# aerius-labs/zksnap-circuits-halo2

Hardware: AMD Instinct MI355X
Metric: BN254 G1 MSM Mpoints/sec (higher is better)
Workload: dtype u32x9 (254-bit modular integer, radix 2^29); 1 GPU; BN254 G1 MSM, 2^20 random points/scalars per GPU (BASELINE configs[1]), point-range sharded x1, inputs resident in HBM, bases registered once (prepared fixed-base table, as under ParamsKZG::commit); points_per_gpu=1048576, parallelism=point-range shard x1 + all_gather(96 B) + fold

## Files before the change

zksnap_circuits_halo2_amd/csrc/msm.hip:

```cpp
#include <hip/hip_runtime.h>
#include <atomic>
#include <cstdint>
#include <cstdio>
#include <cstring>
#include <cstdlib>
#include <mutex>
#include "ec_quad.hpp"
#include "fe_inverse.hpp"
#include "zkhip_internal.hpp"

namespace zkhip {

static inline size_t align_up(size_t v, size_t a) { return (v + a - 1) / a * a; }

constexpr int FINE_BITS = 12;
constexpr int MAX_GROUPS = 128;
constexpr int MAX_WIDE_W = 16;
struct win_layout { int c, W, narrow; };
__host__ __device__ __forceinline__ int win_bits(const win_layout& L, int w) { return w < L.W - L.narrow ? L.c : L.c - 1; }
__host__ __device__ __forceinline__ int win_off(const win_layout& L, int w) { const int full = L.W - L.narrow; return w <= full ? w * L.c : full * L.c + (w - full) * (L.c - 1); }
static int msm_narrow_windows(int c, int W) {
  if (c <= 16) return 0;
  const int narrow = W * c - 256;
  return narrow > 0 && narrow <= W ? narrow : 0;
}
constexpr int MAX_TASK_LEN = 128;
constexpr int TASK_SHIFT = 6;

__device__ __forceinline__ xyzz load_xyzz(const uint32_t* base, size_t idx) {
  const uint4* q = reinterpret_cast<const uint4*>(base + idx * 36);
  uint32_t w[36];
#pragma unroll
  for (int i = 0; i < 9; i++) {
    uint4 v = q[i];
    w[4 * i] = v.x; w[4 * i + 1] = v.y; w[4 * i + 2] = v.z; w[4 * i + 3] = v.w;
  }
  xyzz r;
#pragma unroll
  for (int i = 0; i < 9; i++) { r.X.l[i] = w[i]; r.Y.l[i] = w[9 + i]; r.ZZ.l[i] = w[18 + i]; r.ZZZ.l[i] = w[27 + i]; }
  return r;
}

__device__ __forceinline__ void store_xyzz(uint32_t* base, size_t idx, const xyzz& a) {
  uint32_t w[36];
#pragma unroll
  for (int i = 0; i < 9; i++) { w[i] = a.X.l[i]; w[9 + i] = a.Y.l[i]; w[18 + i] = a.ZZ.l[i]; w[27 + i] = a.ZZZ.l[i]; }
  uint4* q = reinterpret_cast<uint4*>(base + idx * 36);
#pragma unroll
  for (int i = 0; i < 9; i++) q[i] = make_uint4(w[4 * i], w[4 * i + 1], w[4 * i + 2], w[4 * i + 3]);
}

__device__ __forceinline__ xyzz xyzz_shfl_xor(const xyzz& a, int mask) {
  xyzz r;
#pragma unroll
  for (int i = 0; i < NL; i++) {
    r.X.l[i] = (uint32_t)__shfl_xor((int)a.X.l[i], mask, 64);
    r.Y.l[i] = (uint32_t)__shfl_xor((int)a.Y.l[i], mask, 64);
    r.ZZ.l[i] = (uint32_t)__shfl_xor((int)a.ZZ.l[i], mask, 64);
    r.ZZZ.l[i] = (uint32_t)__shfl_xor((int)a.ZZZ.l[i], mask, 64);
  }
  return r;
}

__device__ __forceinline__ fe load_fe9_generic(const uint32_t* p, size_t idx) {
  fe r;
#pragma unroll
  for (int i = 0; i < 9; i++) r.l[i] = p[idx * 9 + i];
  return r;
}
__device__ __forceinline__ void store_fe9_generic(uint32_t* p, size_t idx, const fe& a) {
#pragma unroll
  for (int i = 0; i < 9; i++) p[idx * 9 + i] = a.l[i];
}

__global__ void __launch_bounds__(256) k_digits(const uint32_t* __restrict__ scalars, int16_t* __restrict__ digits,
                                                uint32_t n, uint32_t n_pad, int c, int W, uint32_t K, size_t scalar_stride, int narrow) {
  const size_t idx = (size_t)blockIdx.x * blockDim.x + threadIdx.x;
  if (idx >= (size_t)K * n_pad) return;
  const uint32_t kb = (uint32_t)(idx / n_pad), i = (uint32_t)(idx % n_pad);
  digits += (size_t)kb * n_pad;
  const size_t row = (size_t)K * n_pad;
  if (i >= n) {
    for (int win = 0; win < W; win++) digits[(size_t)win * row + i] = 0;
    return;
  }
  uint32_t w[8];
  load_words(scalars + ((size_t)kb * scalar_stride + i) * 8, w);
  fe c32;
#pragma unroll
  for (int k = 0; k < NL; k++) c32.l[k] = FrParams::FROM_EXT_CANON[k];
  fe s = fe_canon_lt2p<FrParams>(fe_mul<FrParams>(c32, fe_unpack<0>(w)));
  fe_pack(s, w);
  const win_layout lay{c, W, narrow};
  uint32_t carry = 0;
  for (int win = 0; win < W; win++) {
    const int bit = win_off(lay, win), cw = win_bits(lay, win);
    const uint32_t half = 1u << (cw - 1), mask = (1u << cw) - 1;
    uint32_t v = 0;
    if (bit < 256) {
      int wi = bit >> 5, sh = bit & 31;
      uint64_t two = w[wi];
      if (wi + 1 < 8) two |= (uint64_t)w[wi + 1] << 32;
      v = (uint32_t)(two >> sh) & mask;
    }
    v += carry;
    int32_t d;
    if (v >= half) { d = (int32_t)v - (int32_t)(1u << cw); carry = 1; } else { d = (int32_t)v; carry = 0; }
    digits[(size_t)win * row + i] = (int16_t)d;
  }
}

__global__ void __launch_bounds__(1024) k_digits_wide(const uint32_t* __restrict__ scalars, int32_t* __restrict__ digits, uint32_t n, uint32_t n_pad,
                                                       int c, int W, uint32_t* __restrict__ gcount, int narrow) {
  __shared__ uint32_t cnt[MAX_WIDE_W * MAX_GROUPS];
  for (uint32_t t = threadIdx.x; t < (uint32_t)W * MAX_GROUPS; t += blockDim.x) cnt[t] = 0;
  __syncthreads();
  const win_layout lay{c, W, narrow};
  for (uint32_t i = blockIdx.x * blockDim.x + threadIdx.x; i < n_pad; i += gridDim.x * blockDim.x) {
    if (i >= n) {
      for (int win = 0; win < W; win++) digits[(size_t)win * n_pad + i] = 0;
      continue;
    }
    uint32_t w[8];
    load_words(scalars + (size_t)i * 8, w);
    fe c32;
#pragma unroll
    for (int k = 0; k < NL; k++) c32.l[k] = FrParams::FROM_EXT_CANON[k];
    fe sv = fe_canon_lt2p<FrParams>(fe_mul<FrParams>(c32, fe_unpack<0>(w)));
    fe_pack(sv, w);
    uint32_t carry = 0;
    for (int win = 0; win < W; win++) {
      const int bit = win_off(lay, win), cw = win_bits(lay, win);
      const uint32_t half = 1u << (cw - 1), mask = (1u << cw) - 1;
      uint32_t v = 0;
      if (bit < 256) {
        const int wi = bit >> 5, sh = bit & 31;
        uint64_t two = w[wi];
        if (wi + 1 < 8) two |= (uint64_t)w[wi + 1] << 32;
        v = (uint32_t)(two >> sh) & mask;
      }
      v += carry;
      int32_t d;
      if (v >= half) { d = (int32_t)v - (int32_t)(1u << cw); carry = 1; } else { d = (int32_t)v; carry = 0; }
      digits[(size_t)win * n_pad + i] = d;
      if (d != 0) atomicAdd(&cnt[win * MAX_GROUPS + (((uint32_t)(d < 0 ? -d : d) - 1) >> FINE_BITS)], 1u);
    }
  }
  __syncthreads();
  for (uint32_t t = threadIdx.x; t < (uint32_t)W * MAX_GROUPS; t += blockDim.x)
    if (cnt[t]) atomicAdd(&gcount[t], cnt[t]);
}

namespace glv {
__device__ constexpr uint32_t G1[3] = {0xc7e0b3d7u, 0xd91d232eu, 0x2u};
__device__ constexpr uint32_t G2[5] = {0x391eb18eu, 0x7a7bd9d4u, 0xa773d2cfu, 0x4ccef014u, 0x2u};
__device__ constexpr uint32_t A1[2] = {0x94d213e3u, 0x89d32568u};
__device__ constexpr uint32_t A2[4] = {0x1221250bu, 0x0be4e154u, 0xeeb859fdu, 0x6f4d8248u};
__device__ constexpr uint32_t NB1[4] = {0x7d4f1128u, 0x8211bbebu, 0xeeb859fcu, 0x6f4d8248u};
__device__ constexpr uint32_t BETA_EXT[8] = {0xd782e155u, 0x71930c11u, 0xffbe3323u, 0xa6bb947cu, 0xd4741444u, 0xaa303344u, 0x26594943u, 0x2c3b3f0du};

template <int NA, int NB, int NO>
// ... 820 lines not shown

__device__ __forceinline__ xyzz workgroup_sum_128(xyzz acc, uint32_t* __restrict__ xch) {
#pragma unroll 1
  for (uint32_t half = 64; half >= 1; half >>= 1) {
    __syncthreads();
    if (threadIdx.x >= half && threadIdx.x < 2 * half) store_xyzz(xch, threadIdx.x - half, acc);
    __syncthreads();
    if (threadIdx.x < half) acc = xyzz_add(acc, load_xyzz(xch, threadIdx.x));
  }
  return acc;
}

__device__ __forceinline__ void combine_heavy_buckets(uint32_t wg, const uint32_t* __restrict__ task_off, uint32_t* __restrict__ partials,
                                                      uint32_t* __restrict__ buckets, const uint32_t* __restrict__ heavy_count,
                                                      const uint2* __restrict__ heavy, uint32_t heavy_cap, uint32_t* __restrict__ heavy_done,
                                                      uint32_t* __restrict__ xch , uint32_t quad_max) {
  __shared__ uint32_t is_last;
  const uint32_t nh = min(*heavy_count, heavy_cap);
  for (uint32_t i = wg; i < nh; i += HEAVY_WGS) {
    const uint2 e = heavy[i];
    const uint32_t k = e.x, sl = e.y, t = task_off[k], m = task_off[k + 1] - t;
    const uint32_t P = (m + HEAVY_SLICE - 1) / HEAVY_SLICE, lo = sl * HEAVY_SLICE, hi = min(m, lo + HEAVY_SLICE);
    if (m <= quad_max) {
      const uint32_t q = threadIdx.x & 3, quad = threadIdx.x >> 2;
      xyzz acc = xyzz_identity();
#pragma unroll 1
      for (uint32_t j = quad; j < m; j += 32) acc = xyzz_add_quad(acc, load_xyzz(partials, t + j), q);
#pragma unroll 1
      for (int mask = 4; mask < 64; mask <<= 1) acc = xyzz_add_quad(acc, xyzz_shfl_xor(acc, mask), q);
      __syncthreads();
      if (threadIdx.x == 64) store_xyzz(xch, 0, acc);
      __syncthreads();
      if (threadIdx.x < 4) {
        acc = xyzz_add_quad(acc, load_xyzz(xch, 0), q);
        if (q == 0) store_xyzz(buckets, k, acc);
      }
      continue;
    }
    xyzz acc = xyzz_identity();
#pragma unroll 1
    for (uint32_t j = lo + threadIdx.x; j < hi; j += 128) acc = xyzz_add(acc, load_xyzz(partials, t + j));
    acc = workgroup_sum_128(acc, xch);
    if (P == 1) {
      if (threadIdx.x == 0) store_xyzz(buckets, k, acc);
      continue;
    }
    if (threadIdx.x == 0) {
      store_xyzz(partials, t + lo, acc);
      __threadfence();
      is_last = atomicAdd(&heavy_done[i - sl], 1u) == P - 1;
    }
    __syncthreads();
    if (!is_last) continue;
    __threadfence();
    acc = xyzz_identity();
#pragma unroll 1
    for (uint32_t j = threadIdx.x; j < P; j += 128) acc = xyzz_add(acc, load_xyzz(partials, t + j * HEAVY_SLICE));
    acc = workgroup_sum_128(acc, xch);
    if (threadIdx.x == 0) store_xyzz(buckets, k, acc);
  }
}

template <int COMBINE_LANES>
__global__ void __launch_bounds__(128) k_combine_seq(const uint32_t* __restrict__ task_off, uint32_t nbuckets,
                                                     uint32_t* __restrict__ partials, uint32_t* __restrict__ buckets,
                                                     uint32_t seq_parts, uint32_t blocks, const uint32_t* __restrict__ heavy_count,
                                                     const uint2* __restrict__ heavy, uint32_t heavy_cap, uint32_t* __restrict__ heavy_done, uint32_t quad_max) {
  __shared__ __attribute__((aligned(16))) uint32_t xch[64 * 36];
  if (blockIdx.x >= blocks) { combine_heavy_buckets(blockIdx.x - blocks, task_off, partials, buckets, heavy_count, heavy, heavy_cap, heavy_done, xch, quad_max); return; }
  const uint32_t gid = blockIdx.x * blockDim.x + threadIdx.x;
  const uint32_t k = gid / COMBINE_LANES, q = gid % COMBINE_LANES;
  const bool live = k < nbuckets;
  xyzz acc = xyzz_identity();
  uint32_t m = 0;
  if (live) {
    const uint32_t t = task_off[k];
    m = task_off[k + 1] - t;
    const uint32_t left = (m == 1 || m > seq_parts) ? 0u : m;
#pragma unroll 1
    for (uint32_t j = q; j < left; j += COMBINE_LANES) acc = xyzz_add(acc, load_xyzz(partials, t + j));
  }
#pragma unroll 1
  for (int mask = 1; mask < COMBINE_LANES; mask <<= 1) acc = xyzz_add(acc, xyzz_shfl_xor(acc, mask));
  if (live && q == 0 && m != 1 && m <= seq_parts) store_xyzz(buckets, k, acc);
}

template <int COMBINE_LANES>
__global__ void __launch_bounds__(128) k_combine_seq_quad(const uint32_t* __restrict__ task_off, uint32_t nbuckets,
                                                          uint32_t* __restrict__ partials, uint32_t* __restrict__ buckets,
                                                          uint32_t seq_parts, uint32_t blocks, const uint32_t* __restrict__ heavy_count,
                                                          const uint2* __restrict__ heavy, uint32_t heavy_cap, uint32_t* __restrict__ heavy_done, uint32_t quad_max) {
  __shared__ __attribute__((aligned(16))) uint32_t xch[64 * 36];
  if (blockIdx.x >= blocks) { combine_heavy_buckets(blockIdx.x - blocks, task_off, partials, buckets, heavy_count, heavy, heavy_cap, heavy_done, xch, quad_max); return; }
  const uint32_t gid = blockIdx.x * blockDim.x + threadIdx.x;
  const uint32_t q = gid & 3, lane = (gid >> 2) % COMBINE_LANES, k = (gid >> 2) / COMBINE_LANES;
  const bool live = k < nbuckets;
  xyzz acc = xyzz_identity();
  uint32_t m = 0;
  if (live) {
    const uint32_t t = task_off[k];
    m = task_off[k + 1] - t;
    const uint32_t left = (m == 1 || m > seq_parts) ? 0u : m;
#pragma unroll 1
    for (uint32_t j = lane; j < left; j += COMBINE_LANES) acc = xyzz_add_quad(acc, load_xyzz(partials, t + j), q);
  }
#pragma unroll 1
  for (int mask = 1; mask < COMBINE_LANES; mask <<= 1) acc = xyzz_add_quad(acc, xyzz_shfl_xor(acc, 4 * mask), q);
  if (live && lane == 0 && q == 0 && m != 1 && m <= seq_parts) store_xyzz(buckets, k, acc);
}

__global__ void __launch_bounds__(128) k_pyramid_step(const uint32_t* __restrict__ in, uint32_t* __restrict__ out,
                                                      uint32_t N, int s, uint32_t in_stride, uint32_t out_stride) {
  const uint32_t per_win = N / 2 + (uint32_t)s * (N / 4);
  const int win = blockIdx.y;
  const uint32_t* wi = in + (size_t)win * in_stride * 36;
  uint32_t* wo = out + (size_t)win * out_stride * 36;
#pragma unroll 1
  for (uint32_t tid = blockIdx.x * blockDim.x + threadIdx.x; tid < per_win; tid += gridDim.x * blockDim.x) {
    uint32_t ia, ib;
    if (tid < N / 2) {
      ia = 2 * tid; ib = 2 * tid + 1;
    } else {
      uint32_t r = tid - N / 2;
      uint32_t l = r / (N / 4), u = r % (N / 4);
      if ((int)l == s - 1) { ia = 4 * u + 1; ib = 4 * u + 3; }
      else { ia = N + l * (N / 2) + 2 * u; ib = ia + 1; }
    }
    store_xyzz(wo, tid, xyzz_add(load_xyzz(wi, ia), load_xyzz(wi, ib)));
  }
}

__global__ void __launch_bounds__(128) k_pyramid_step_quad(const uint32_t* __restrict__ in, uint32_t* __restrict__ out,
                                                           uint32_t N, int s, uint32_t in_stride, uint32_t out_stride) {
  const uint32_t per_win = N / 2 + (uint32_t)s * (N / 4);
  const uint32_t gid = blockIdx.x * blockDim.x + threadIdx.x;
  const uint32_t tid = gid >> 2, q = gid & 3;
  if (tid >= per_win) return;
  const int win = blockIdx.y;
  const uint32_t* wi = in + (size_t)win * in_stride * 36;
  uint32_t* wo = out + (size_t)win * out_stride * 36;
  uint32_t ia, ib;
  if (tid < N / 2) {
    ia = 2 * tid; ib = 2 * tid + 1;
  } else {
    uint32_t r = tid - N / 2;
    uint32_t l = r / (N / 4), u = r % (N / 4);
    if ((int)l == s - 1) { ia = 4 * u + 1; ib = 4 * u + 3; }
    else { ia = N + l * (N / 2) + 2 * u; ib = ia + 1; }
  }
  const xyzz r = xyzz_add_quad(load_xyzz(wi, ia), load_xyzz(wi, ib), q);
  if (q == 0) store_xyzz(wo, tid, r);
}

__global__ void __launch_bounds__(64) k_window_horner(const uint32_t* __restrict__ in, uint32_t in_stride, int nz,
                                                      uint32_t* __restrict__ winsum, int W) {
  const int gid = blockIdx.x * blockDim.x + threadIdx.x;
  const int win = gid >> 5, lane = gid & 31;
  xyzz acc = xyzz_identity();
  if (win < W) {
    const uint32_t* wi = in + (size_t)win * in_stride * 36;
    int dbl = 0;
    if (lane < nz) { acc = load_xyzz(wi, 2 + lane); dbl = lane; }
    else if (lane == nz) { acc = load_xyzz(wi, 1); dbl = nz; }
    else if (lane == nz + 1) acc = xyzz_add(load_xyzz(wi, 0), load_xyzz(wi, 1));
#pragma unroll 1
    for (int i = 0; i < dbl; i++) acc = xyzz_dbl(acc);
  }
#pragma unroll 1
  for (int mask = 1; mask < 32; mask <<= 1) acc = xyzz_add(acc, xyzz_shfl_xor(acc, mask));
  if (win < W && lane == 0) store_xyzz(winsum, win, acc);
}

__global__ void __launch_bounds__(128) k_window_horner_quad(const uint32_t* __restrict__ in, uint32_t in_stride, int nz,
                                                            uint32_t* __restrict__ winsum, uint32_t* __restrict__ jac_out) {
  __shared__ __attribute__((aligned(16))) uint32_t xch[36];
  const int win = blockIdx.x, term = threadIdx.x >> 2;
  const uint32_t q = threadIdx.x & 3;
  const uint32_t* wi = in + (size_t)win * in_stride * 36;
  xyzz acc = xyzz_identity();
  int dbl = 0;
  if (term < nz) { acc = load_xyzz(wi, 2 + term); dbl = term; }
  else if (term == nz) { acc = load_xyzz(wi, 1); dbl = nz; }
  else if (term == nz + 1) acc = xyzz_add_quad(load_xyzz(wi, 0), load_xyzz(wi, 1), q);
#pragma unroll 1
  for (int i = 0; i < dbl; i++) acc = xyzz_dbl_quad(acc, q);
#pragma unroll 1
  for (int mask = 4; mask < 64; mask <<= 1) acc = xyzz_add_quad(acc, xyzz_shfl_xor(acc, mask), q);
  if (threadIdx.x == 64) store_xyzz(xch, 0, acc);
  __syncthreads();
  if (threadIdx.x < 4) {
    acc = xyzz_add_quad(acc, load_xyzz(xch, 0), q);
    if (q == 0) {
      if (jac_out) store_jacobian(acc, jac_out + (size_t)win * 24);
      else store_xyzz(winsum, win, acc);
    }
  }
}

__global__ void __launch_bounds__(64) k_fold(const uint32_t* __restrict__ winsum, int W, int c, uint32_t* __restrict__ out) {
  if (threadIdx.x >= 4 || blockIdx.x != 0) return;
  const uint32_t q = threadIdx.x;
  xyzz acc = load_xyzz(winsum, W - 1);
  for (int w = W - 2; w >= 0; w--) {
#pragma unroll 1
    for (int i = 0; i < c; i++) acc = xyzz_dbl_quad(acc, q);
    acc = xyzz_add_quad(acc, load_xyzz(winsum, w), q);
  }
  if (q == 0) store_jacobian(acc, out);
}

__global__ void __launch_bounds__(64) k_store_results(const uint32_t* __restrict__ winsum, uint32_t K, uint32_t* __restrict__ out) {
  const uint32_t k = blockIdx.x * blockDim.x + threadIdx.x;
  if (k < K) store_jacobian(load_xyzz(winsum, k), out + (size_t)k * 24);
}

__global__ void __launch_bounds__(64) k_sum_jacobian(const uint32_t* __restrict__ in, int m, uint32_t* __restrict__ out, uint32_t stride) {
  const uint32_t q = threadIdx.x & 3;
  const int grp = threadIdx.x >> 2;
  in += (size_t)blockIdx.x * 24;
  out += (size_t)blockIdx.x * 24;
  xyzz acc = xyzz_identity();
  for (int i = grp; i < m; i += 16) acc = xyzz_add_quad(acc, load_jacobian(in + (size_t)i * stride * 24), q);
#pragma unroll 1
  for (int mask = 4; mask < 64; mask <<= 1) {
    if ((mask >> 2) >= m && mask > 4) break;
    acc = xyzz_add_quad(acc, xyzz_shfl_xor(acc, mask), q);
  }
  if (threadIdx.x == 0) store_jacobian(acc, out);
}

static bool msm_top_window_is_degenerate(int c) {
  const int W = (256 + c - 1) / c, top_bits = 254 - (W - 1) * c;
  return top_bits > 0 && top_bits < 6;
}

static inline int msm_windows(int c, bool glv) {
  if (!glv) return (256 + c - 1) / c;
  return (128 + c - 1) / c + ((c == 2 || c == 4) ? 1 : 0);
}

int msm_pick_window(size_t n) {
  int best = 16;
  double best_cost = 1e300;
  for (int c = 2; c <= 16; c++) {
    const int Wi = msm_windows(c, true), top_bits = 127 - (Wi - 1) * c;
    if (top_bits > 0 && top_bits < 6) continue;
    const double cost = (double)Wi * (10.0 * (double)(2 * n) + 28.0 * (double)(1u << (c - 1)));
    if (cost < best_cost) { best_cost = cost; best = c; }
  }
  return best;
}


constexpr int MAX_WINDOW_PREPARED = 20;

int msm_pick_window_prepared(size_t n) {
  const bool large = n >= ((size_t)1 << 20);
  int best = 2;
  double best_cost = 1e300;
  for (int c = 2; c <= MAX_WINDOW_PREPARED; c++) {
    const double W = (256 + c - 1) / c, buckets = (double)(1u << (c - 1));
    if (msm_top_window_is_degenerate(c) && c <= 16) continue;
    if (c > 16 && !large) continue;
    if (c == 17) continue;
    double cost;
    if (!large) cost = W * 10.0 * (double)n + 28.0 * buckets;
    else {
      const double eff = c == 20 ? 1.0 : (c == 19 ? 1.13 : (c == 18 ? 1.06 : 1.07));
      cost = W * (10.0 * eff + 1.0) * (double)n + 39.0 * buckets + 1.1e6 * (double)(c - 2) + 13.0e6;
    }
    if (cost < best_cost) { best_cost = cost; best = c; }
  }
  if (n >= ((size_t)1 << 14) && n < ((size_t)3 << 14)) best = 15;
  return best;
}

struct msm_layout {
  uint32_t task_shift;
  size_t max_tasks;
  void* digits;
  uint32_t* stage_ref; uint16_t* stage_fine;
  char* zero_lo; size_t zero_bytes;
  uint32_t *gcounters, *counters, *count, *sorted, *offset, *cursor, *task_off, *bsum1, *bsum2;
  task_t* tasks; uint4* order;
  uint32_t *partials, *pyrA, *pyrB, *winsum;
  uint32_t* endo;
  int combine_lanes;
  uint32_t seq_parts;
  uint2* heavy; uint32_t heavy_cap;
  uint32_t* heavy_done;
  size_t total;
};

static uint32_t msm_task_shift(size_t entries , size_t NB, size_t xyzz_bytes = 144) {
  uint32_t task_shift = TASK_SHIFT;
  if ((entries >> 7) >= ((size_t)3 << 16)) task_shift = 7;
  const bool g2 = xyzz_bytes == 288;
  if ((entries >> TASK_SHIFT) < ((size_t)1 << (g2 ? 14 : 17))) {
    const double occ = (double)entries / (double)NB;
    double best = 1e300;
    for (uint32_t sh = 2; sh <= (uint32_t)TASK_SHIFT; sh++) {
      const double L = (double)(1u << sh), parts = occ / L;
      const double est = 5.0 * L + (g2 ? 15.0 : 10.0) * (parts > 1.0 ? parts - 1.0 : 0.0);
      if (est < best) { best = est; task_shift = sh; }
    }
  }
  return task_shift;
}

constexpr size_t GLV_TWO_LEVEL_MIN = (size_t)1 << 18;
constexpr size_t PREP_TWO_LEVEL_MIN = (size_t)1 << 16;
static bool msm_two_level(int c, bool glv, size_t n_in, bool shared_buckets, size_t K) {
  if (c > 16) return true;
  if (c != 16 || K != 1) return false;
  if (glv) return n_in >= GLV_TWO_LEVEL_MIN;
  return shared_buckets && n_in >= PREP_TWO_LEVEL_MIN;
}

static msm_layout msm_lay_out(char* base, size_t n_in, size_t K, int c, bool prepared, size_t xyzz_bytes = 144, bool glv = false) {
  msm_layout L;
  const size_t n = glv ? 2 * n_in : n_in;
  const size_t W = (size_t)msm_windows(c, glv), B = (size_t)1 << (c - 1), WB = prepared ? K : W, NB = WB * B;
  const bool wide = msm_two_level(c, glv, n_in, prepared, K);
  const size_t nk = n * K, entries = W * nk;
  const size_t n_pad = (n + 7) & ~(size_t)7;
  L.task_shift = msm_task_shift(entries, NB, xyzz_bytes);
  L.max_tasks = (entries >> L.task_shift) + NB + 1;
  const double parts_avg = (double)entries / (double)NB / (double)(1u << L.task_shift);
  L.combine_lanes = parts_avg <= 2.0 ? 1 : (parts_avg <= 4.0 ? 2 : (parts_avg <= 12.0 ? 4 : 8));
  L.seq_parts = 16u * (uint32_t)L.combine_lanes;
  L.heavy_cap = (uint32_t)(std::min<size_t>(L.max_tasks / (L.seq_parts + 1) + 1, NB) + L.max_tasks / HEAVY_SLICE + 1);
  char* p = base;
  auto carve = [&](size_t bytes) { void* r = p; p += align_up(bytes, 256); return r; };
  L.digits = carve(W * K * n_pad * (wide ? sizeof(int32_t) : sizeof(int16_t)));
  L.stage_ref = wide ? (uint32_t*)carve(entries * sizeof(uint32_t)) : nullptr;
  L.stage_fine = wide ? (uint16_t*)carve(entries * sizeof(uint16_t)) : nullptr;
  L.zero_lo = p;
  L.gcounters = wide ? (uint32_t*)carve(32768) : nullptr;
  L.counters = (uint32_t*)carve(2048);
  L.count = (uint32_t*)carve((NB + 1) * sizeof(uint32_t));
  L.heavy_done = (uint32_t*)carve((size_t)L.heavy_cap * sizeof(uint32_t));
  L.zero_bytes = (size_t)(p - L.zero_lo);
  L.sorted = (uint32_t*)carve(entries * sizeof(uint32_t));
  L.offset = (uint32_t*)carve((NB + 1) * sizeof(uint32_t));
  L.cursor = (uint32_t*)carve((NB + 1) * sizeof(uint32_t));
  L.task_off = (uint32_t*)carve((NB + 1) * sizeof(uint32_t));
  L.heavy = (uint2*)carve((size_t)L.heavy_cap * sizeof(uint2));
  L.bsum1 = (uint32_t*)carve((NB / SCAN_TILE + 2) * sizeof(uint32_t));
// ... 29 lines not shown
                    size_t xyzz_bytes, void* ws, size_t ws_bytes, hipStream_t stream, msm_tasks_view* out, bool glv) {
  const uint32_t K = (uint32_t)batch;
  const bool wide = msm_two_level(c, glv, n_in, shared_buckets, batch);
  const int W = msm_windows(c, glv);
  if (glv && (K != 1 || c > 16 || shared_buckets)) { set_error("msm: GLV digits are for one vector of the general path"); return ZKHIP_EINVAL; }
  const size_t n = glv ? 2 * n_in : n_in;
  const uint32_t B = 1u << (c - 1);
  const int WB = shared_buckets ? (int)K : W;
  const uint32_t NB = (uint32_t)WB * B;
  if ((size_t)W * n * K >= (1ull << 32) || (size_t)WB * B >= (1ull << 31)) { set_error("msm: W*n*batch overflows 32-bit slot index"); return ZKHIP_EINVAL; }
  if (c > 16 && (!shared_buckets || K != 1)) { set_error("msm: windows above 16 bits need one shared bucket set"); return ZKHIP_EINVAL; }
  if (wide && !shared_buckets && (size_t)W * (B >> FINE_BITS) > (size_t)MAX_GROUPS) { set_error("msm: two-level sort: %d windows x %u groups exceed %d", W, B >> FINE_BITS, MAX_GROUPS); return ZKHIP_EINVAL; }
  if (wide && W > MAX_WIDE_W) { set_error("msm: %d windows of %d bits exceed the wide path's %d", W, c, MAX_WIDE_W); return ZKHIP_EINVAL; }
  const msm_layout lay = msm_lay_out((char*)ws, n_in, K, c, shared_buckets, xyzz_bytes, glv);
  if (ws_bytes < lay.total) { set_error("msm: workspace too small (%zu < %zu bytes)", ws_bytes, lay.total); return ZKHIP_EINVAL; }
  const uint32_t task_shift = lay.task_shift;
  const uint32_t n_pad = (uint32_t)((n + 7) & ~(size_t)7);
  void* const digits = lay.digits;
  uint32_t* const stage_ref = lay.stage_ref;
  uint16_t* const stage_fine = lay.stage_fine;
  uint32_t *const gcounters = lay.gcounters, *const counters = lay.counters, *const count = lay.count, *const sorted = lay.sorted,
           *const offset = lay.offset, *const cursor = lay.cursor, *const task_off = lay.task_off, *const bsum1 = lay.bsum1, *const bsum2 = lay.bsum2;
  task_t* const tasks = lay.tasks;
  uint4* const order = lay.order;

  prof_begin(stream);
  HIPCHK(hipMemsetAsync(lay.zero_lo, 0, lay.zero_bytes, stream));
  const size_t sstride = K > 1 ? scalar_stride : n;
  const size_t nk = n * K, max_tasks = lay.max_tasks;
  (void)nk; (void)max_tasks;
  const unsigned dblocks = (unsigned)(((size_t)K * n_pad + 255) / 256);
  const int narrow = (shared_buckets && !glv) ? msm_narrow_windows(c, W) : 0;
  if (glv && wide) hipLaunchKernelGGL(k_digits_glv<int32_t>, dim3((unsigned)((std::max<size_t>(n_in, 8) + 255) / 256)), dim3(256), 0, stream, d_scalars, (int32_t*)digits, (uint32_t)n_in, n_pad, c, W);
  else if (glv) hipLaunchKernelGGL(k_digits_glv<int16_t>, dim3((unsigned)((std::max<size_t>(n_in, 8) + 255) / 256)), dim3(256), 0, stream, d_scalars, (int16_t*)digits, (uint32_t)n_in, n_pad, c, W);
  else if (wide) {
    const unsigned wg_cap = n_pad > (1u << 21) ? 1024u : 512u;
    const unsigned wblocks = (unsigned)std::min<size_t>(((size_t)n_pad + 1023) / 1024, wg_cap);
    hipLaunchKernelGGL(k_digits_wide, dim3(wblocks), dim3(1024), 0, stream, d_scalars, (int32_t*)digits, (uint32_t)n, n_pad, c, W, gcounters + 1024, narrow);
  }
  else hipLaunchKernelGGL(k_digits, dim3(dblocks), dim3(256), 0, stream, d_scalars, (int16_t*)digits, (uint32_t)n, n_pad, c, W, K, sstride, 0);
  prof_mark(stream, "digits");
  uint32_t chunks = (uint32_t)((n + 65535) / 65536);
  while (chunks * (uint32_t)W * K < 256 && chunks < (n + 4095) / 4096) chunks *= 2;
  if (chunks == 0) chunks = 1;
  const uint32_t chunk = (uint32_t)((((n + chunks - 1) / chunks) + 7) & ~(size_t)7);
  const size_t lds = wide ? ((size_t)4 << FINE_BITS) : (size_t)B * sizeof(uint32_t);
  static std::once_flag attr_once[64];
  static hipError_t attr_err[64];
  int cur_dev = 0;
  HIPCHK(hipGetDevice(&cur_dev));
  std::call_once(attr_once[cur_dev & 63], [&] {
    hipError_t e = hipFuncSetAttribute((const void*)k_sort_pass<false>, hipFuncAttributeMaxDynamicSharedMemorySize, 128 * 1024);
    if (e == hipSuccess) e = hipFuncSetAttribute((const void*)k_sort_pass<true>, hipFuncAttributeMaxDynamicSharedMemorySize, 128 * 1024);
    if (e == hipSuccess) e = hipFuncSetAttribute((const void*)k_fine_sorted, hipFuncAttributeMaxDynamicSharedMemorySize, (2 * (1 << FINE_BITS) + SORT_CHUNK + SORT_CHUNK / 16) * 4);
    attr_err[cur_dev & 63] = e;
  });
  HIPCHK(attr_err[cur_dev & 63]);
  const uint32_t gstride = (wide && !shared_buckets) ? (B >> FINE_BITS) : 0u;
  const int G = wide ? (int)(gstride ? (uint32_t)W * gstride : (B >> FINE_BITS)) : 1;
  const uint32_t sort_chunk = SORT_CHUNK;
  const uint32_t sort_chunks = (uint32_t)(((size_t)W * n + sort_chunk - 1) / sort_chunk) + (uint32_t)G;
  const uint32_t wb_stride = shared_buckets ? 0u : B;
  if (wide) {
    if (glv)
      hipLaunchKernelGGL(k_coarse_count, dim3(chunks, W), dim3(1024), 0, stream, (const int32_t*)digits, n_pad, chunk, gcounters + 1024, gstride);
    hipLaunchKernelGGL(k_group_offsets, dim3(1), dim3(64), 0, stream, gcounters + 1024, W, G, gcounters + 128, gcounters + 3072, gcounters + 512, sort_chunk);
    static_assert(MAX_GROUPS == 128, "k_coarse_sorted scans two groups per lane of one wavefront");
    hipLaunchKernelGGL(k_coarse_sorted, dim3((n_pad + COARSE_CHUNK - 1) / COARSE_CHUNK, W), dim3(1024), 0, stream, (const int32_t*)digits, n_pad, gcounters + 3072,
                       stage_ref, stage_fine, ref_base, ref_stride, gstride);
    prof_mark(stream, "coarse");
    hipLaunchKernelGGL(k_fine_count, dim3(sort_chunks), dim3(1024), 0, stream, stage_fine, gcounters + 128, gcounters + 512, G, count, sort_chunk);
  } else {
    hipLaunchKernelGGL(k_sort_pass<false>, dim3(chunks, W, K), dim3(1024), lds, stream, (const int16_t*)digits, n_pad, chunk, c, count, (uint32_t*)nullptr, wb_stride, ref_base, ref_stride);
  }
  prof_mark(stream, "count");
  const uint32_t nblk = (NB + SCAN_TILE - 1) / SCAN_TILE;
  const bool scan_single = NB <= SCAN_SINGLE_MAX;
  if (scan_single) {
    hipLaunchKernelGGL(k_scan_single<0>, dim3(1), dim3(1024), 0, stream, count, (uint32_t)NB, counters + 0, offset, cursor, 0u, (uint32_t*)nullptr);
  } else {
    hipLaunchKernelGGL(k_scan_sums2, dim3(nblk), dim3(SCAN_BLOCK), 0, stream, count, NB, bsum1, bsum2, task_shift);
    hipLaunchKernelGGL(k_scan_top2, dim3(1), dim3(SCAN_BLOCK), 0, stream, bsum1, bsum2, nblk, counters + 0, counters + 1);
    hipLaunchKernelGGL(k_scan_apply2, dim3(std::min(nblk, SCAN_APPLY_WGS)), dim3(SCAN_BLOCK), 0, stream, count, NB, bsum1, bsum2, counters + 0, counters + 1, offset, cursor, task_off,
                       task_shift, nblk, counters + 32);
  }
  prof_mark(stream, "scan");
  if (wide) {
    hipLaunchKernelGGL(k_fine_sorted, dim3(sort_chunks), dim3(1024), (size_t)(2u * (1u << FINE_BITS) + SORT_CHUNK + SORT_CHUNK / 16) * 4, stream, stage_fine, stage_ref,
                       gcounters + 128, gcounters + 512, G, cursor, sorted);
  }
  else hipLaunchKernelGGL(k_sort_pass<true>, dim3(chunks, W, K), dim3(1024), lds, stream, (const int16_t*)digits, n_pad, chunk, c, cursor, sorted, wb_stride, ref_base, ref_stride);
  prof_mark(stream, "scatter");
  const unsigned task_blocks = (unsigned)std::min<size_t>((NB + 255) / 256, 256);
  if (scan_single) {
    hipLaunchKernelGGL(k_scan_single<1>, dim3(1), dim3(1024), 0, stream, count, (uint32_t)NB, counters + 1, task_off, (uint32_t*)nullptr, task_shift, counters + 192);
    hipLaunchKernelGGL(k_make_tasks, dim3(task_blocks), dim3(256), 0, stream, offset, task_off, NB, tasks, task_shift, counters + 2, lay.seq_parts,
                       counters + 3, lay.heavy, lay.heavy_cap);
    hipLaunchKernelGGL(k_make_order, dim3(task_blocks), dim3(256), 0, stream, offset, task_off, NB, task_shift, counters + 192, sorted, order,
                       (const uint32_t*)nullptr, (task_t*)nullptr, counters + 2, lay.seq_parts, counters + 3, lay.heavy, lay.heavy_cap);
  } else {
    hipLaunchKernelGGL(k_make_order, dim3(task_blocks), dim3(256), 0, stream, offset, task_off, NB, task_shift, counters + 192, sorted, order,
                       (const uint32_t*)(counters + 32), tasks, counters + 2, lay.seq_parts, counters + 3, lay.heavy, lay.heavy_cap);
  }
  prof_mark(stream, "tasks");
  out->c = c; out->W = W; out->WB = WB; out->B = B; out->NB = NB; out->task_shift = task_shift; out->max_tasks = lay.max_tasks; out->nk = n * K;
  out->tasks = tasks; out->ntasks = counters + 1; out->max_parts = counters + 2; out->order = order; out->sorted = sorted; out->task_off = task_off;
  out->partials = lay.partials; out->pyrA = lay.pyrA; out->pyrB = lay.pyrB; out->winsum = lay.winsum;
  out->combine_lanes = lay.combine_lanes; out->seq_parts = lay.seq_parts; out->heavy_count = counters + 3; out->heavy = lay.heavy; out->heavy_cap = lay.heavy_cap; out->heavy_done = lay.heavy_done;
  out->endo = lay.endo;
  HIPCHK(hipGetLastError());
  return ZKHIP_OK;
}

static int msm_accumulate_combine(const msm_tasks_view& tv, const uint32_t* d_bases, bool prepared, bool glv, size_t n, uint32_t* buckets, hipStream_t stream) {
  const uint32_t NB = tv.NB;
  const size_t max_tasks = tv.max_tasks;
  const task_t* const tasks = tv.tasks;
  uint32_t* const counters = tv.ntasks - 1;
  const uint4* const order = tv.order;
  const uint32_t *const sorted = tv.sorted, *const task_off = tv.task_off;
  uint32_t* const partials = tv.partials;
  {
    uint32_t blocks = (uint32_t)((max_tasks + 127) / 128);
    if (blocks > 256 * 64) blocks = 256 * 64;
    if (prepared) hipLaunchKernelGGL(k_accumulate<true>, dim3(blocks), dim3(128), 0, stream, tasks, counters + 1, order, sorted, d_bases, partials, buckets, (const uint32_t*)nullptr, 0xffffffffu);
    else hipLaunchKernelGGL(k_accumulate<false>, dim3(blocks), dim3(128), 0, stream, tasks, counters + 1, order, sorted, d_bases, partials, buckets, (const uint32_t*)tv.endo,
                            glv ? (uint32_t)n : 0xffffffffu);
  }
  prof_mark(stream, "accumulate");
  {
    const int combine_lanes = tv.combine_lanes;
    const uint32_t seq_parts = tv.seq_parts;
    const size_t lanes_total = (size_t)NB * combine_lanes;
    const bool quad = lanes_total * 4 <= 131072;
    const unsigned blocks = (unsigned)((lanes_total * (quad ? 4 : 1) + 127) / 128);
#define ZK_LAUNCH_COMBINE(L)                                                                                                                        \
    do {                                                                                                                                              \
      if (quad) hipLaunchKernelGGL(k_combine_seq_quad<L>, dim3(blocks + HEAVY_WGS), dim3(128), 0, stream, task_off, NB, partials, buckets, seq_parts, blocks,   \
                                   tv.heavy_count, (const uint2*)tv.heavy, tv.heavy_cap, tv.heavy_done, HEAVY_QUAD_MAX);                              \
      else hipLaunchKernelGGL(k_combine_seq<L>, dim3(blocks + HEAVY_WGS), dim3(128), 0, stream, task_off, NB, partials, buckets, seq_parts, blocks,             \
                              tv.heavy_count, (const uint2*)tv.heavy, tv.heavy_cap, tv.heavy_done, HEAVY_QUAD_MAX);                                   \
    } while (0)
    if (combine_lanes == 1) ZK_LAUNCH_COMBINE(1);
    else if (combine_lanes == 2) ZK_LAUNCH_COMBINE(2);
    else if (combine_lanes == 4) ZK_LAUNCH_COMBINE(4);
    else ZK_LAUNCH_COMBINE(8);
#undef ZK_LAUNCH_COMBINE
  }
  prof_mark(stream, "combine");
  return ZKHIP_OK;
}

static int msm_reduce_buckets(int WB, uint32_t B, int c, uint32_t K, bool prepared, uint32_t* cur, uint32_t* nxt, uint32_t* winsum, uint32_t* d_out, hipStream_t stream) {
  constexpr size_t PYR_QUAD_MAX = 65536;
  uint32_t in_stride = B;
  int nz = 0;
  {
    uint32_t N = B;
    int s = 1;
    while (N > 2) {
      uint32_t per_win = N / 2 + (uint32_t)s * (N / 4);
      uint32_t out_stride = per_win;
      if ((size_t)per_win * WB <= PYR_QUAD_MAX) hipLaunchKernelGGL(k_pyramid_step_quad, dim3((4 * per_win + 127) / 128, WB), dim3(128), 0, stream, cur, nxt, N, s, in_stride, out_stride);
      else hipLaunchKernelGGL(k_pyramid_step, dim3((per_win + 127) / 128, WB), dim3(128), 0, stream, cur, nxt, N, s, in_stride, out_stride);
      uint32_t* t = cur; cur = nxt; nxt = t;
      in_stride = out_stride;
      N >>= 1;
      s++;
    }
    nz = s - 1;
  }
  prof_mark(stream, "pyramid");
  if (B == 1) { set_error("msm: internal: B == 1"); return ZKHIP_EINVAL; }
  const bool direct = prepared && WB <= 2048;
  if (WB <= 2048) hipLaunchKernelGGL(k_window_horner_quad, dim3(WB), dim3(128), 0, stream, cur, in_stride, nz, winsum, direct ? d_out : (uint32_t*)nullptr);
  else hipLaunchKernelGGL(k_window_horner, dim3((WB * 32 + 63) / 64), dim3(64), 0, stream, cur, in_stride, nz, winsum, WB);
  prof_mark(stream, "horner");
  if (prepared) { if (!direct) hipLaunchKernelGGL(k_store_results, dim3((K + 63) / 64), dim3(64), 0, stream, winsum, K, d_out); }
  else hipLaunchKernelGGL(k_fold, dim3(1), dim3(64), 0, stream, winsum, WB, c, d_out);
  prof_mark(stream, "fold");
  HIPCHK(hipGetLastError());
  return ZKHIP_OK;
}

int msm_g1_device(const uint32_t* d_scalars, const uint32_t* d_bases, size_t n, uint32_t* d_out, void* ws, size_t ws_bytes,
                  int c_override, hipStream_t stream, const prepared_bases* prepared, size_t prepared_off, size_t batch,
                  size_t scalar_stride) {
  if (batch == 0) return ZKHIP_OK;
  if (n == 0) {
    for (size_t k = 0; k < batch; k++) hipLaunchKernelGGL(k_sum_jacobian, dim3(1), dim3(64), 0, stream, (const uint32_t*)nullptr, 0, d_out + k * 24, 1u);
    HIPCHK(hipGetLastError());
    return ZKHIP_OK;
  }
  if (batch > 1 && (!prepared || prepared->c > 16 || batch > 65535)) { set_error("msm: batch needs prepared bases with a window <= 16 bits"); return ZKHIP_EINVAL; }
  const uint32_t K = (uint32_t)batch;
  if (n >= (1ull << 31)) { set_error("msm: n = %zu too large", n); return ZKHIP_EINVAL; }
  const int c = prepared ? prepared->c : (c_override > 0 ? c_override : msm_pick_window(n));
  if (c < 2 || c > (prepared ? MAX_WINDOW_PREPARED : 16)) { set_error("msm: window bits %d out of range", c); return ZKHIP_EINVAL; }
  if (prepared) {
    if (prepared_off + n > prepared->n) { set_error("msm: range exceeds the prepared bases"); return ZKHIP_EINVAL; }
    if ((size_t)((256 + c - 1) / c) * prepared->n >= (1ull << 31)) { set_error("msm: prepared table too large for 31-bit point references"); return ZKHIP_EINVAL; }
    d_bases = prepared->table;
    if (prepared->direct && batch == 1) return msm_g1_direct(d_scalars, n, prepared, prepared_off, d_out, ws, ws_bytes, stream);
  }
  msm_tasks_view tv;
  const bool glv = msm_uses_glv(prepared != nullptr, batch);
  int rc = msm_build_tasks(d_scalars, n, batch, scalar_stride, c, prepared != nullptr, prepared ? (uint32_t)prepared_off : 0u, prepared ? (uint32_t)prepared->n : 0u,
                           144, ws, ws_bytes, stream, &tv, glv);
  if (rc != ZKHIP_OK) return rc;
  if (glv) hipLaunchKernelGGL(k_endo_bases, dim3((unsigned)((n + 255) / 256)), dim3(256), 0, stream, d_bases, (uint32_t)n, tv.endo);
  if ((rc = msm_accumulate_combine(tv, d_bases, prepared != nullptr, glv, n, tv.pyrA, stream)) != ZKHIP_OK) return rc;
  return msm_reduce_buckets(tv.WB, tv.B, c, K, prepared != nullptr, tv.pyrA, tv.pyrB, tv.winsum, d_out, stream);
}

__global__ void __launch_bounds__(128) k_bucket_sets_add(uint32_t* __restrict__ acc, const uint32_t* __restrict__ add, uint32_t nb) {
  const uint32_t k = blockIdx.x * blockDim.x + threadIdx.x;
  if (k >= nb) return;
  store_xyzz(acc, k, xyzz_add(load_xyzz(acc, k), load_xyzz(add, k)));
}

static size_t msm_chunk_lay_bytes(size_t chunk_cap, int c) {
  size_t b = msm_lay_out(nullptr, chunk_cap, 1, c, true).total;
  if (chunk_cap > 1) b = std::max(b, msm_lay_out(nullptr, chunk_cap - 1, 1, c, true).total);
  return align_up(b, 256);
}

size_t msm_chunk_workspace_bytes(size_t chunk_cap, int c) {
  if (chunk_cap == 0) return 0;
  return msm_chunk_lay_bytes(chunk_cap, c) + align_up(((size_t)1 << (c - 1)) * 144, 256);
}

int msm_chunk_add(const uint32_t* d_scalars, size_t n, const prepared_bases* pb, size_t pb_off, size_t chunk_cap, bool first, void* ws, size_t ws_bytes, hipStream_t stream) {
  if (!pb || n == 0 || n > chunk_cap || pb_off + n > pb->n) { set_error("msm_chunk_add: bad piece (n = %zu, capacity %zu)", n, chunk_cap); return ZKHIP_EINVAL; }
  const size_t lay_bytes = msm_chunk_lay_bytes(chunk_cap, pb->c);
  if (ws_bytes < msm_chunk_workspace_bytes(chunk_cap, pb->c)) { set_error("msm_chunk_add: workspace too small"); return ZKHIP_EINVAL; }
  uint32_t* const acc = (uint32_t*)((char*)ws + lay_bytes);
  msm_tasks_view tv;
  int rc = msm_build_tasks(d_scalars, n, 1, 0, pb->c, true, (uint32_t)pb_off, (uint32_t)pb->n, 144, ws, lay_bytes, stream, &tv, false);
  if (rc != ZKHIP_OK) return rc;
  if ((rc = msm_accumulate_combine(tv, pb->table, true, false, n, first ? acc : tv.pyrA, stream)) != ZKHIP_OK) return rc;
  if (!first) hipLaunchKernelGGL(k_bucket_sets_add, dim3((tv.NB + 127) / 128), dim3(128), 0, stream, acc, (const uint32_t*)tv.pyrA, tv.NB);
  HIPCHK(hipGetLastError());
  return ZKHIP_OK;
}

int msm_chunk_finish(const prepared_bases* pb, size_t chunk_cap, uint32_t* d_out, void* ws, size_t ws_bytes, hipStream_t stream) {
  if (!pb || ws_bytes < msm_chunk_workspace_bytes(chunk_cap, pb->c)) { set_error("msm_chunk_finish: workspace too small"); return ZKHIP_EINVAL; }
  const msm_layout lay = msm_lay_out((char*)ws, chunk_cap, 1, pb->c, true);
  uint32_t* const acc = (uint32_t*)((char*)ws + msm_chunk_lay_bytes(chunk_cap, pb->c));
  return msm_reduce_buckets(1, 1u << (pb->c - 1), pb->c, 1, true, acc, lay.pyrA, lay.winsum, d_out, stream);
}


constexpr int GEN_CHUNK = 32;

__device__ __forceinline__ xyzz scalar_mul_affine(const uint32_t (&kw)[8], const fe& gx, const fe& gy) {
  xyzz acc = xyzz_identity();
  for (int bit = 255; bit >= 0; bit--) {
    acc = xyzz_dbl(acc);
    if ((kw[bit >> 5] >> (bit & 31)) & 1) xyzz_madd(acc, gx, gy);
  }
  return acc;
}

__device__ __forceinline__ fe fq_inverse(const fe& a) { return fe_inverse<Fq>(a); }

__global__ void __launch_bounds__(64) k_gen_walk(const uint32_t* __restrict__ t0_d ,
                                                 uint32_t n, uint32_t* __restrict__ out, uint32_t* __restrict__ tmp_pts,
                                                 uint32_t* __restrict__ tmp_pref) {
  const uint32_t j = blockIdx.x * blockDim.x + threadIdx.x;
  const uint32_t lo = j * GEN_CHUNK;
  if (lo >= n) return;
  const uint32_t cnt = min((uint32_t)GEN_CHUNK, n - lo);
  uint32_t w0[8], wd[8], kw[8];
#pragma unroll
  for (int i = 0; i < 8; i++) { w0[i] = t0_d[i]; wd[i] = t0_d[8 + i]; }
  fe one_r = fe_one<FrParams>();
  fe t0 = fe_mul<FrParams>(one_r, fe_from_ext_lazy(w0));
  fe dd = fe_mul<FrParams>(one_r, fe_from_ext_lazy(wd));
  fe lo_f = fe_zero();
  lo_f.l[0] = lo & LMASK; lo_f.l[1] = lo >> LB;
  fe r2; 
#pragma unroll
  for (int i = 0; i < NL; i++) r2.l[i] = FrParams::R2[i];
  fe lo_m = fe_mul<FrParams>(r2, lo_f);
  fe k = fe_norm(fe_add(t0, fe_mul<FrParams>(lo_m, dd)));
  fe raw1;
#pragma unroll
  for (int i = 0; i < NL; i++) raw1.l[i] = FrParams::RAW_ONE[i];
  fe kc = fe_canon_lt2p<FrParams>(fe_mul<FrParams>(raw1, k));
  fe_pack(kc, kw);
  fe dc = fe_canon_lt2p<FrParams>(fe_mul<FrParams>(raw1, dd));
  uint32_t dw[8];
  fe_pack(dc, dw);
  fe gx = fe_one<Fq>();
  fe gy = fe_norm(fe_dbl(gx));
  xyzz P = scalar_mul_affine(kw, gx, gy);
  xyzz D = scalar_mul_affine(dw, gx, gy);
  fe pref = fe_one<Fq>();
  for (uint32_t i = 0; i < cnt; i++) {
    store_xyzz(tmp_pts, lo + i, P);
    store_fe9_generic(tmp_pref, lo + i, pref);
    if (!xyzz_is_identity(P)) pref = fe_mul<Fq>(pref, fe_mul<Fq>(P.ZZ, P.ZZZ));
    P = xyzz_add(P, D);
  }
  fe inv = fq_inverse(pref);
  for (uint32_t ii = cnt; ii-- > 0;) {
    xyzz Q = load_xyzz(tmp_pts, lo + ii);
    uint32_t* o = out + (size_t)(lo + ii) * 16;
    if (xyzz_is_identity(Q)) {
#pragma unroll
      for (int t = 0; t < 16; t++) o[t] = 0;
      continue;
    }
    fe pre = load_fe9_generic(tmp_pref, lo + ii);
    fe winv = fe_mul<Fq>(inv, pre);
    inv = fe_mul<Fq>(inv, fe_mul<Fq>(Q.ZZ, Q.ZZZ));
    fe x = fe_mul<Fq>(fe_mul<Fq>(winv, Q.ZZZ), Q.X);
    fe y = fe_mul<Fq>(fe_mul<Fq>(winv, Q.ZZ), Q.Y);
    uint32_t wx[8], wy[8];
    fe_to_ext<Fq>(x, wx);
    fe_to_ext<Fq>(y, wy);
#pragma unroll
    for (int t = 0; t < 8; t++) { o[t] = wx[t]; o[8 + t] = wy[t]; }
  }
}

static void fr_pow2_montgomery(int e, uint32_t out[8]) {
  static const uint64_t RMOD[4] = {0x43e1f593f0000001ull, 0x2833e84879b97091ull, 0xb85045b68181585dull, 0x30644e72e131a029ull};
// ... 593 lines not shown
```

Measured before the change: 771.4 Mpoints/s.

## Fuse bucket pyramid tail levels and Horner into one LDS-resident finish kernel

Adds a reduction planner that picks kernels for each pyramid level. When there are few window sets (at most 64), the last small pyramid levels and the per-window Horner/doubling combine are fused into a single 512-thread kernel that keeps intermediates in shared memory. A new pair kernel also merges two pyramid levels into one launch using lane shuffles. The aim is to remove many tiny kernel launches and global round trips at the low-occupancy tail of the bucket reduction. The cost is extra complexity, a planner that can reject some configurations, and one workgroup per window during the finish stage.

```diff
diff --git a/zksnap_circuits_halo2_amd/csrc/msm.hip b/zksnap_circuits_halo2_amd/csrc/msm.hip
--- a/zksnap_circuits_halo2_amd/csrc/msm.hip
+++ b/zksnap_circuits_halo2_amd/csrc/msm.hip
@@ -7,6 +7,7 @@
 #include <mutex>
 #include "ec_quad.hpp"
 #include "fe_inverse.hpp"
+#include "reduce_plan.hpp"
 #include "zkhip_internal.hpp"
 
 namespace zkhip {
@@ -1133,6 +1134,30 @@
   if (q == 0) store_xyzz(wo, tid, r);
 }
 
+__global__ void __launch_bounds__(128) k_pyramid_pair_quad(const uint32_t* __restrict__ in, uint32_t* __restrict__ out,
+                                                           uint32_t N, int s, uint32_t in_stride, uint32_t out_stride) {
+  const uint32_t outs = N / 4 + (uint32_t)(s + 1) * (N / 8);
+  const uint32_t gid = blockIdx.x * blockDim.x + threadIdx.x;
+  const uint32_t o = gid >> 3, half = (gid >> 2) & 1, q = gid & 3;
+  if (o >= outs) return;
+  const int win = blockIdx.y;
+  const uint32_t* wi = in + (size_t)win * in_stride * 36;
+  uint32_t* wo = out + (size_t)win * out_stride * 36;
+  uint32_t ia, ib;
+  if (o < N / 4) {
+    ia = 4 * o + 2 * half; ib = ia + 1;
+  } else {
+    const uint32_t r = o - N / 4;
+    const uint32_t l = r / (N / 8), v = r % (N / 8);
+    if ((int)l == s - 1) { ia = 8 * v + 4 * half + 1; ib = ia + 2; }
+    else if ((int)l == s) { ia = 8 * v + 4 * half + 2; ib = ia + 1; }
+    else { ia = N + l * (N / 2) + 4 * v + 2 * half; ib = ia + 1; }
+  }
+  const xyzz p = xyzz_add_quad(load_xyzz(wi, ia), load_xyzz(wi, ib), q);
+  const xyzz r = xyzz_add_quad(p, xyzz_shfl_xor(p, 4), q);
+  if ((gid & 7) == 0) store_xyzz(wo, o, r);
+}
+
 __global__ void __launch_bounds__(64) k_window_horner(const uint32_t* __restrict__ in, uint32_t in_stride, int nz,
                                                       uint32_t* __restrict__ winsum, int W) {
   const int gid = blockIdx.x * blockDim.x + threadIdx.x;
@@ -1175,6 +1200,81 @@
       if (jac_out) store_jacobian(acc, jac_out + (size_t)win * 24);
       else store_xyzz(winsum, win, acc);
     }
+  }
+}
+
+constexpr int FINISH_THREADS = 512;
+constexpr int FINISH_CHAIN0 = 11, FINISH_CHAIN1 = 15, FINISH_CHAIN2 = 17;
+
+__global__ void __launch_bounds__(FINISH_THREADS) k_reduce_finish(const uint32_t* __restrict__ in, uint32_t in_stride, uint32_t N, int s,
+                                                                  uint32_t* __restrict__ winsum, uint32_t* __restrict__ jac_out) {
+  __shared__ __attribute__((aligned(16))) uint32_t lds[(REDUCE_FINISH_ADDS + REDUCE_FINISH_ADDS2) * 36];
+  __shared__ __attribute__((aligned(16))) uint32_t xch[3 * 36];
+  constexpr uint32_t BUF1 = REDUCE_FINISH_ADDS * 36;
+  const int win = blockIdx.x;
+  const uint32_t q = threadIdx.x & 3, quad = threadIdx.x >> 2;
+  const uint32_t* wi = in + (size_t)win * in_stride * 36;
+  const bool levels = N > 2;
+  uint32_t cur = 0;
+  bool first = true;
+#pragma unroll 1
+  while (N > 2) {
+    const uint32_t per_win = N / 2 + (uint32_t)s * (N / 4);
+    const uint32_t nxt = first ? 0u : (cur == 0 ? BUF1 : 0u);
+    static_assert(FINISH_THREADS / 4 >= (int)REDUCE_FINISH_ADDS, "one quad per addition of the widest level");
+    if (quad < per_win) {
+      uint32_t ia, ib;
+      if (quad < N / 2) {
+        ia = 2 * quad; ib = 2 * quad + 1;
+      } else {
+        const uint32_t r = quad - N / 2;
+        const uint32_t l = r / (N / 4), u = r % (N / 4);
+        if ((int)l == s - 1) { ia = 4 * u + 1; ib = 4 * u + 3; }
+        else { ia = N + l * (N / 2) + 2 * u; ib = ia + 1; }
+      }
+      xyzz a, b;
+      if (first) { a = load_xyzz(wi, ia); b = load_xyzz(wi, ib); }
+      else { a = load_xyzz(lds + cur, ia); b = load_xyzz(lds + cur, ib); }
+      const xyzz r = xyzz_add_quad(a, b, q);
+      if (q == 0) store_xyzz(lds + nxt, quad, r);
+    }
+    __syncthreads();
+    cur = nxt; first = false;
+    N >>= 1;
+    s++;
+  }
+  const int nz = s - 1;
+  const int wave = threadIdx.x >> 6, j = (threadIdx.x & 63) >> 2;
+  const int n0 = min(nz, FINISH_CHAIN0) + 1;
+  int dbl = 0;
+  int idx = -1;
+  int count = 0;
+  auto chains = [&](int lo, int hi) {
+    count = max(0, min(nz, hi) - lo + 1);
+    if (j < count) { dbl = lo + j; idx = dbl < nz ? 2 + dbl : 1; }
+  };
+  if (wave == 0) { chains(0, FINISH_CHAIN0); count = n0 + 2; if (j == n0) idx = 0; else if (j == n0 + 1) idx = 1; }
+  else if (wave == 1) chains(FINISH_CHAIN0 + 1, FINISH_CHAIN1);
+  else if (wave == 2) chains(FINISH_CHAIN1 + 1, FINISH_CHAIN2);
+  else if (wave == 3) chains(FINISH_CHAIN2 + 1, 63);
+  xyzz acc = xyzz_identity();
+  if (idx >= 0) { if (levels) acc = load_xyzz(lds + cur, idx); else acc = load_xyzz(wi, idx); }
+#pragma unroll 1
+  for (int i = 0; i < dbl; i++) acc = xyzz_dbl_quad(acc, q);
+#pragma unroll 1
+  for (int phase = 0; phase < 2; phase++) {
+    if (phase == 1) {
+      __syncthreads();
+      count = wave == 0 ? 4 : 0;
+      if (wave == 0 && j >= 1) acc = j < 4 ? load_xyzz(xch, j - 1) : xyzz_identity();
+    }
+#pragma unroll 1
+    for (int mask = 4; (mask >> 2) < count; mask <<= 1) acc = xyzz_add_quad(acc, xyzz_shfl_xor(acc, mask), q);
+    if (phase == 0 && wave >= 1 && wave <= 3 && (threadIdx.x & 63) == 0) store_xyzz(xch, wave - 1, acc);
+  }
+  if (threadIdx.x == 0) {
+    if (jac_out) store_jacobian(acc, jac_out + (size_t)win * 24);
+    else store_xyzz(winsum, win, acc);
   }
 }
 
@@ -1510,29 +1610,27 @@
 }
 
 static int msm_reduce_buckets(int WB, uint32_t B, int c, uint32_t K, bool prepared, uint32_t* cur, uint32_t* nxt, uint32_t* winsum, uint32_t* d_out, hipStream_t stream) {
-  constexpr size_t PYR_QUAD_MAX = 65536;
-  uint32_t in_stride = B;
-  int nz = 0;
-  {
-    uint32_t N = B;
-    int s = 1;
-    while (N > 2) {
-      uint32_t per_win = N / 2 + (uint32_t)s * (N / 4);
-      uint32_t out_stride = per_win;
-      if ((size_t)per_win * WB <= PYR_QUAD_MAX) hipLaunchKernelGGL(k_pyramid_step_quad, dim3((4 * per_win + 127) / 128, WB), dim3(128), 0, stream, cur, nxt, N, s, in_stride, out_stride);
-      else hipLaunchKernelGGL(k_pyramid_step, dim3((per_win + 127) / 128, WB), dim3(128), 0, stream, cur, nxt, N, s, in_stride, out_stride);
-      uint32_t* t = cur; cur = nxt; nxt = t;
-      in_stride = out_stride;
-      N >>= 1;
-      s++;
-    }
-    nz = s - 1;
-  }
-  prof_mark(stream, "pyramid");
   if (B == 1) { set_error("msm: internal: B == 1"); return ZKHIP_EINVAL; }
+  reduce_plan plan;
+  if (!reduce_make_plan(B, WB, &plan)) { set_error("msm: internal: no reduction plan for %u buckets x %d sets", B, WB); return ZKHIP_EINVAL; }
   const bool direct = prepared && WB <= 2048;
-  if (WB <= 2048) hipLaunchKernelGGL(k_window_horner_quad, dim3(WB), dim3(128), 0, stream, cur, in_stride, nz, winsum, direct ? d_out : (uint32_t*)nullptr);
-  else hipLaunchKernelGGL(k_window_horner, dim3((WB * 32 + 63) / 64), dim3(64), 0, stream, cur, in_stride, nz, winsum, WB);
+  for (int i = 0; i < plan.n; i++) {
+    const reduce_launch& L = plan.l[i];
+    if (L.kind == REDUCE_FINISH) {
+      prof_mark(stream, "pyramid");
+      hipLaunchKernelGGL(k_reduce_finish, dim3(WB), dim3(FINISH_THREADS), 0, stream, cur, L.in_stride, L.N, L.s, winsum, direct ? d_out : (uint32_t*)nullptr);
+      break;
+    }
+    if (L.kind == REDUCE_STEP) hipLaunchKernelGGL(k_pyramid_step, dim3((L.out_stride + 127) / 128, WB), dim3(128), 0, stream, cur, nxt, L.N, L.s, L.in_stride, L.out_stride);
+    else if (L.kind == REDUCE_STEP_QUAD) hipLaunchKernelGGL(k_pyramid_step_quad, dim3((4 * L.out_stride + 127) / 128, WB), dim3(128), 0, stream, cur, nxt, L.N, L.s, L.in_stride, L.out_stride);
+    else hipLaunchKernelGGL(k_pyramid_pair_quad, dim3((8 * L.out_stride + 127) / 128, WB), dim3(128), 0, stream, cur, nxt, L.N, L.s, L.in_stride, L.out_stride);
+    uint32_t* t = cur; cur = nxt; nxt = t;
+  }
+  if (!plan.finish) {
+    prof_mark(stream, "pyramid");
+    if (WB <= 2048) hipLaunchKernelGGL(k_window_horner_quad, dim3(WB), dim3(128), 0, stream, cur, plan.last_stride, plan.nz, winsum, direct ? d_out : (uint32_t*)nullptr);
+    else hipLaunchKernelGGL(k_window_horner, dim3((WB * 32 + 63) / 64), dim3(64), 0, stream, cur, plan.last_stride, plan.nz, winsum, WB);
+  }
   prof_mark(stream, "horner");
   if (prepared) { if (!direct) hipLaunchKernelGGL(k_store_results, dim3((K + 63) / 64), dim3(64), 0, stream, winsum, K, d_out); }
   else hipLaunchKernelGGL(k_fold, dim3(1), dim3(64), 0, stream, winsum, WB, c, d_out);
diff --git a/zksnap_circuits_halo2_amd/csrc/reduce_plan.hpp b/zksnap_circuits_halo2_amd/csrc/reduce_plan.hpp
--- /dev/null
+++ b/zksnap_circuits_halo2_amd/csrc/reduce_plan.hpp
@@ -0,0 +1,70 @@
+#pragma once
+#include <cstddef>
+#include <cstdint>
+
+namespace zkhip {
+
+constexpr size_t REDUCE_QUAD_MAX = 65536;
+constexpr size_t REDUCE_PAIR_MAX_LANES = (size_t)1 << 16;
+constexpr int REDUCE_FINISH_MAX_SETS = 64;
+constexpr uint32_t REDUCE_FINISH_ADDS = 128;
+constexpr uint32_t REDUCE_FINISH_ADDS2 = 80;
+constexpr int REDUCE_MAX_LAUNCHES = 32;
+
+enum reduce_kind : int { REDUCE_STEP = 0, REDUCE_STEP_QUAD = 1, REDUCE_PAIR_QUAD = 2, REDUCE_FINISH = 3 };
+
+struct reduce_launch {
+  int kind;
+  int s;
+  int steps;
+  uint32_t N;
+  uint32_t in_stride;
+  uint32_t out_stride;
+};
+
+struct reduce_plan {
+  int n;
+  int nz;
+  bool finish;
+  uint32_t last_stride;
+  reduce_launch l[REDUCE_MAX_LAUNCHES];
+};
+
+inline uint32_t reduce_step_adds(uint32_t N, int s) { return N / 2 + (uint32_t)s * (N / 4); }
+inline uint32_t reduce_state_elems(uint32_t N, int s) { return N + (uint32_t)(s - 1) * (N / 2); }
+
+inline bool reduce_make_plan(uint32_t B, int WB, reduce_plan* p) {
+  p->n = 0;
+  p->finish = WB <= REDUCE_FINISH_MAX_SETS;
+  uint32_t N = B, stride = B;
+  int s = 1;
+  while (N > 2) {
+    const uint32_t adds = reduce_step_adds(N, s);
+    if (p->finish && adds <= REDUCE_FINISH_ADDS) break;
+    if (p->n >= REDUCE_MAX_LAUNCHES - 1) return false;
+    reduce_launch& L = p->l[p->n++];
+    L.s = s; L.N = N; L.in_stride = stride;
+    const uint32_t adds2 = N >= 8 ? reduce_step_adds(N / 2, s + 1) : 0;
+    const bool pair = p->finish && N >= 8 && adds2 > REDUCE_FINISH_ADDS
+                      && (size_t)adds2 * (size_t)WB * 8 < REDUCE_PAIR_MAX_LANES;
+    if ((size_t)adds * (size_t)WB > REDUCE_QUAD_MAX) { L.kind = REDUCE_STEP; L.steps = 1; L.out_stride = adds; }
+    else if (pair) { L.kind = REDUCE_PAIR_QUAD; L.steps = 2; L.out_stride = adds2; }
+    else { L.kind = REDUCE_STEP_QUAD; L.steps = 1; L.out_stride = adds; }
+    stride = L.out_stride;
+    N >>= L.steps;
+    s += L.steps;
+  }
+  if (p->finish) {
+    if (N > 2 && (reduce_step_adds(N, s) > REDUCE_FINISH_ADDS || (N > 4 && reduce_step_adds(N / 2, s + 1) > REDUCE_FINISH_ADDS2))) return false;
+    reduce_launch& L = p->l[p->n++];
+    L.kind = REDUCE_FINISH; L.s = s; L.N = N; L.in_stride = stride; L.out_stride = 0;
+    L.steps = 0;
+    for (uint32_t M = N; M > 2; M >>= 1) L.steps++;
+    s += L.steps;
+  }
+  p->nz = s - 1;
+  p->last_stride = stride;
+  return true;
+}
+
+}
```

New measurement: 786.4 Mpoints/s (median of 6 runs). 1.02x the previous value.
